# ZhendongWang6/Uformer

Hardware: AMD Instinct MI355X
Metric: restored images/sec (256x256, Uformer-B) (higher is better)
Workload: dtype bf16

## Files before the change

uformer_amd/csrc/uf_attnblk.hip:

```cpp
#include <stdlib.h>

#include <atomic>
#include <type_traits>

#include "uf_internal.h"

namespace uf {
namespace {

struct AttnBlkParams {
    float* x; int ld;
    float* xo; int ldo;
    const float* gamma; const float* beta; const float* modulator;
    const void* Wqkv; const float* bqkv;
    const float* rpb_tab;
    const void* Wp; const float* bp;
    const float* gamma2; const float* beta2;
    const void* W1; const float* b1;
    void* h1;
    const float* drop;
    void* s_xn; void* s_q; void* s_k; void* s_vt; void* s_o; void* s_z;
    int n_windows, H, W, shift;
    float qscale;
    float qscale_plain;
    unsigned long long* tbuf;
};

constexpr float LOG2E = 1.4426950408889634f;

#ifndef UF_P1_OFFSET
#define UF_P1_OFFSET 0
#endif
#ifndef UF_FC1_OFFSET
#define UF_FC1_OFFSET 0
#endif
#ifndef UF_STAGGER
#define UF_STAGGER 0
#endif
#ifndef UF_SETPRIO
#define UF_SETPRIO 0
#endif
#define UF_PRIO_UP() do { if (UF_SETPRIO) __builtin_amdgcn_s_setprio(1); } while (0)
#define UF_PRIO_DN() do { if (UF_SETPRIO) __builtin_amdgcn_s_setprio(0); } while (0)
#ifndef UF_ABL
#define UF_ABL 0
#endif
#ifndef UF_NT
#define UF_NT 0
#endif
#ifndef UF_LN_ROTATE
#define UF_LN_ROTATE 0
#endif
#ifndef UF_LN_WIDE
#define UF_LN_WIDE 1
#endif
#ifndef UF_QKV_RING
#define UF_QKV_RING 3
#endif
#ifndef UF_PROJ_RING
#define UF_PROJ_RING 3
#endif
#ifndef UF_FC1_RING
#define UF_FC1_RING 5
#endif
#ifndef UF_HOIST
#define UF_HOIST 7
#endif
template <int C> constexpr bool hoist_on() { return (C <= 128 && (UF_HOIST & 1)) || (C == 256 && (UF_HOIST & 2)) || (C == 512 && (UF_HOIST & 4)); }

#ifndef UF_ATTN_LR_DEFAULT
#define UF_ATTN_LR_DEFAULT 0
#endif
template <typename T> struct FragFromAcc {
    static __device__ __forceinline__ void make(Frag<T>& f, f32x4 a, f32x4 b) {
        f.v = u32x4{pack2<T>(a[0], a[1]), pack2<T>(a[2], a[3]), pack2<T>(b[0], b[1]), pack2<T>(b[2], b[3])};
    }
};
template <> struct FragFromAcc<float> {
    static __device__ __forceinline__ void make(Frag<float>& f, f32x4 a, f32x4 b) { f.lo = a; f.hi = b; }
};

template <typename T> __device__ __forceinline__ void wfrag_load(Frag<T>& f, const T* p) {
    if constexpr (UF_ABL == 6 && sizeof(T) == 2) { const unsigned v = 0x3c003c00u ^ (unsigned)(uintptr_t)p; f.v = u32x4{v, v, v, v}; }
    else load_frag(f, p);
}
template <typename T> __device__ __forceinline__ void afrag_load(Frag<T>& f, const T* p) {
    if constexpr (UF_ABL == 7 && sizeof(T) == 2) { const unsigned v = 0x3c003c00u ^ (unsigned)(uintptr_t)p; f.v = u32x4{v, v, v, v}; }
    else load_frag(f, p);
}

template <typename T> __device__ __forceinline__ void pin_frag(Frag<T>& f) {
    if constexpr (sizeof(T) == 2) asm volatile("" : "+v"(f.v));
}

template <int N> __device__ __forceinline__ float tree_sum(float* v) {
    static_assert((N & (N - 1)) == 0, "power of two");
#pragma unroll
    for (int w = 1; w < N; w *= 2)
#pragma unroll
        for (int i = 0; i < N; i += 2 * w) v[i] += v[i + w];
    return v[0];
}

template <typename T, int C, int WAVES, int UW = 4, bool ACT = true>
struct Fc1Walk {
    static_assert(UW == 4 || UW == 2, "units of 64 x 64 or 64 x 32");
    static constexpr int SZ = sizeof(T), KS = C / 32, RING = KS >= 8 ? UF_FC1_RING : (KS >= 4 ? 4 : 3), N4 = 4 * C, UNITS = N4 / (16 * UW);
    const T* wrow[UW];
    Frag<T> wf[RING][UW];
    const T* W1;
    int lane;
    __device__ __forceinline__ void wload(int ks, int slot) {
#pragma unroll
        for (int i = 0; i < UW; ++i) wfrag_load(wf[slot][i], wrow[i] + ks * 512);
    }
    __device__ __forceinline__ void unit_prefetch(int u) {
#pragma unroll
        for (int i = 0; i < UW; ++i) wrow[i] = W1 + ((size_t)(u * UW + i) * KS * 64 + lane) * 8;
#pragma unroll
        for (int s = 0; s < RING - 1; ++s)
            if (s < KS) wload(s, s);
    }
    __device__ __forceinline__ void first(const T* W1_, int wave, int lane_) {
        W1 = W1_; lane = lane_;
        if (wave < UNITS) unit_prefetch(wave);
    }
    __device__ __forceinline__ void run(const char* Xn, int SA, const float* b1, T* h1, const WinGeom& geo, int wave) {
    static_assert(SZ == 2, "direct-store epilogue packs pairs of a 2-byte type");
    const int fr = lane & 15, fg = lane >> 4;
    size_t rowoff[4];
#pragma unroll
    for (int j = 0; j < 4; ++j) rowoff[j] = (size_t)window_token(geo, j * 16 + fr) * N4;
    if (WAVES == 8 && UF_FC1_OFFSET > 0 && wave >= 4) __builtin_amdgcn_s_sleep(UF_FC1_OFFSET * (C / 256) > 127 ? 127 : UF_FC1_OFFSET * (C / 256));
#pragma unroll 1
    for (int u = wave; u < UNITS; u += WAVES) {
        const int nbase = u * 16 * UW;
        f32x4 acc[UW][4];
#pragma unroll
        for (int i = 0; i < UW; ++i)
#pragma unroll
            for (int j = 0; j < 4; ++j) acc[i][j] = f32x4{0.f, 0.f, 0.f, 0.f};
        const char* arow = Xn + fr * SA + fg * 8 * SZ;
        Frag<T> af[2][4];
        auto aload = [&](int ks, int slot) {
#pragma unroll
            for (int j = 0; j < 4; ++j) afrag_load(af[slot][j], reinterpret_cast<const T*>(arow + j * 16 * SA + ks * 32 * SZ));
        };
        aload(0, 0);
        f32x4 bv[UW];
#pragma unroll
        for (int i = 0; i < UW; ++i) bv[i] = *reinterpret_cast<const f32x4*>(b1 + nbase + i * 16 + fg * 4);
#pragma unroll
        for (int ks = 0; ks < KS; ++ks) {
            if (ks + RING - 1 < KS) wload(ks + RING - 1, (ks + RING - 1) % RING);
            if (ks + 1 < KS) aload(ks + 1, (ks + 1) & 1);
            __builtin_amdgcn_sched_barrier(0);
            UF_PRIO_UP();
#pragma unroll
            for (int i = 0; i < UW; ++i)
#pragma unroll
                for (int j = 0; j < 4; ++j) mma16(acc[i][j], wf[ks % RING][i], af[ks & 1][j]);
            UF_PRIO_DN();
            __builtin_amdgcn_sched_barrier(0);
        }
        if (u + WAVES < UNITS) unit_prefetch(u + WAVES);
        __builtin_amdgcn_sched_barrier(0);
#pragma unroll
        for (int j = 0; j < 4; ++j) {
#pragma unroll
            for (int ip = 0; ip < UW; ip += 2) {
                f32x4 va = acc[ip][j] + bv[ip], vb = acc[ip + 1][j] + bv[ip + 1];
                if (UF_ABL != 8 && ACT) { gelu4<T>(va); gelu4<T>(vb); }
                const unsigned a0 = pack2<T>(va[0], va[1]), a1 = pack2<T>(va[2], va[3]);
                const unsigned c0 = pack2<T>(vb[0], vb[1]), c1 = pack2<T>(vb[2], vb[3]);
                const u32x2_t s0 = __builtin_amdgcn_permlane16_swap(a0, c0, false, false);
                const u32x2_t s1 = __builtin_amdgcn_permlane16_swap(a1, c1, false, false);
                const int n = nbase + (ip + (fg & 1)) * 16 + (fg >> 1) * 8;
                if (UF_ABL == 4) asm volatile("" :: "v"(s0[0]), "v"(s1[0]), "v"(s0[1]), "v"(s1[1]), "v"(h1 + rowoff[j] + n));
                else if (UF_NT & 1) __builtin_nontemporal_store(u32x4{s0[0], s1[0], s0[1], s1[1]}, reinterpret_cast<u32x4*>(h1 + rowoff[j] + n));
                else *reinterpret_cast<u32x4*>(h1 + rowoff[j] + n) = u32x4{s0[0], s1[0], s0[1], s1[1]};
            }
        }
    }
    }
};

struct NoWalk {
    template <typename... A> __device__ __forceinline__ void first(A...) {}
    template <typename... A> __device__ __forceinline__ void run(A...) {}
};

template <typename T, int C, int NT, int LR = 0, int TR = 0>
__global__ __launch_bounds__(NT, LR == 3 ? 3 : (LR == 1 ? (C <= 32 ? 5 : (C == 64 ? 4 : 3)) : ((sizeof(T) == 2 && C <= 32) ? 4 : ((sizeof(T) == 2 && C == 64) ? 3 : 2)))) void attn_block_kernel(const AttnBlkParams p) {
    constexpr bool ST = LR == 3;
    constexpr int SZ = sizeof(T);
    constexpr int WAVES = NT / 64;
    constexpr int HEADS = C / 32;
    constexpr int SA = C * SZ + 16;
    constexpr int KS = C / 32;
    constexpr int QT = HEADS >= 4 ? 4 : HEADS;
    constexpr int UNITS = HEADS * (4 / QT);
    extern __shared__ __attribute__((aligned(16))) char smem[];
    char* Xn = smem;
    char* Os = ST ? smem : smem + 64 * SA;
    float* Tab = reinterpret_cast<float*>(smem + (ST ? 1 : 2) * 64 * SA);
    float* Red = Tab + HEADS * 225;
    float* Bq = Red + 2 * WAVES * 64;

    const int tid = threadIdx.x, lane = tid & 63;
    const int wave = __builtin_amdgcn_readfirstlane(tid >> 6);
    const int fr = lane & 15, fg = lane >> 4;
    const int bw = blockIdx.x;
    const WinGeom geo = window_geom(bw, p.H, p.W, p.shift);
    auto stamp = [&](int k) {
        if (p.tbuf && lane == 0 && (bw & 63) == 0) p.tbuf[((bw >> 6) * WAVES + wave) * 16 + k] = __builtin_readcyclecounter();
    };
    stamp(0);
    Census census; census.begin();
    if (UF_STAGGER > 0 && ((blockIdx.x >> 8) & 1)) {
#pragma unroll
        for (int k = 0; k < UF_STAGGER; ++k) __builtin_amdgcn_s_sleep(127);
    }

    constexpr int NTABV = HEADS * 225 + 4 * C, NTAB = (NTABV + NT - 1) / NT;
    float tabv[NTAB];
#pragma unroll
    for (int k = 0; k < NTAB; ++k) {
        int i = tid + k * NT;
        i = i < NTABV ? i : NTABV - 1;
        const float* src = i < HEADS * 225 ? p.rpb_tab + i : (i < HEADS * 225 + 3 * C ? p.bqkv + (i - HEADS * 225) : p.bp + (i - HEADS * 225 - 3 * C));
        tabv[k] = *src;
    }
    constexpr bool HOIST = hoist_on<C>() && SZ == 2;
    constexpr int WR = (SZ == 2 && C >= 256) ? UF_QKV_RING : ((SZ == 2 && C >= 128) ? 3 : 2);
    const T* Wqkv = reinterpret_cast<const T*>(p.Wqkv);
    const T* wrow[6];
    Frag<T> wf[WR][LR ? 2 : 6];
    auto wload = [&](int ks, int slot) {
#pragma unroll
        for (int i = 0; i < 6; ++i) wfrag_load(wf[slot][i], wrow[i] + ks * 512);
    };
    auto wload2 = [&](int g, int slot) {
        const int pj = g / KS, ks = g - pj * KS, base = pj == 0 ? 2 : (pj == 1 ? 4 : 0);
#pragma unroll
        for (int i = 0; i < 2; ++i) wfrag_load(wf[slot][i], wrow[base + i] + ks * 512);
    };
    auto unit_weights = [&](int u) {
        const int h = u / (4 / QT);
#pragma unroll
        for (int i = 0; i < 6; ++i) wrow[i] = Wqkv + ((size_t)((i >> 1) * (C / 16) + h * 2 + (i & 1)) * KS * 64 + lane) * 8;
#pragma unroll
        for (int pf = 0; pf < WR - 1; ++pf) {
            if constexpr (LR) { if (pf < 3 * KS) wload2(pf, pf); }
            else { if (pf < KS) wload(pf, pf); }
        }
    };
    if constexpr (HOIST) {
        if (wave < UNITS) unit_weights(wave);
    }
    {
        constexpr int LPR = UF_LN_WIDE ? ((C / 16) < 8 ? 8 : (C / 16)) : ((C / 4) < 64 ? (C / 4) : 64);
        constexpr int V4 = C / (4 * LPR);
        constexpr int RPP = NT / LPR;
        constexpr int NP = 64 / RPP;
        constexpr int U0 = (16 / V4) < NP ? (16 / V4) : NP;
        constexpr int U = (ST && U0 > 2) ? 2 : U0;
        static_assert(NP >= 1 && NP % U == 0, "pass batching");
        const int sub = tid % LPR;
        static_assert((U & (U - 1)) == 0, "U is a power of two");
        const int rot = UF_LN_ROTATE ? bw : 0;
#pragma unroll 1
        for (int r0 = 0; r0 < 64; r0 += RPP * U) {
            f32x4 v[U][V4], md[U][V4];
#pragma unroll
            for (int u = 0; u < U; ++u) {
                const int src = window_token(geo, r0 + ((u + rot) & (U - 1)) * RPP + tid / LPR);
#pragma unroll
                for (int i = 0; i < V4; ++i) {
                    if (UF_ABL == 1) v[u][i] = f32x4{(float)src, (float)i, (float)sub, 1.0f};
                    else if (UF_NT & 4) v[u][i] = __builtin_nontemporal_load(reinterpret_cast<const f32x4*>(p.x + (size_t)src * p.ld + (i * LPR + sub) * 4));
                    else v[u][i] = *reinterpret_cast<const f32x4*>(p.x + (size_t)src * p.ld + (i * LPR + sub) * 4);
                }
            }
            if (p.modulator && UF_ABL != 3) {
#pragma unroll
                for (int u = 0; u < U; ++u) {
                    const int row = r0 + ((u + rot) & (U - 1)) * RPP + tid / LPR;
#pragma unroll
                    for (int i = 0; i < V4; ++i) md[u][i] = *reinterpret_cast<const f32x4*>(p.modulator + (size_t)row * C + (i * LPR + sub) * 4);
                }
            } else {
#pragma unroll
                for (int u = 0; u < U; ++u)
#pragma unroll
                    for (int i = 0; i < V4; ++i) md[u][i] = f32x4{0.f, 0.f, 0.f, 0.f};
            }
            f32x4 gm[V4], bt[V4];
#pragma unroll
            for (int i = 0; i < V4; ++i) {
                gm[i] = *reinterpret_cast<const f32x4*>(p.gamma + (i * LPR + sub) * 4);
                bt[i] = *reinterpret_cast<const f32x4*>(p.beta + (i * LPR + sub) * 4);
            }
#pragma unroll
            for (int u = 0; u < U; ++u) {
                const int row = r0 + ((u + rot) & (U - 1)) * RPP + tid / LPR;
                float sum = 0.f;
#pragma unroll
                for (int i = 0; i < V4; ++i) sum += (v[u][i][0] + v[u][i][1]) + (v[u][i][2] + v[u][i][3]);
                sum = allreduce<RedSum, LPR>(sum);
                const float mean = sum * (1.0f / C);
                float sq = 0.f;
#pragma unroll
                for (int i = 0; i < V4; ++i) {
                    v[u][i] -= mean;
                    sq += (v[u][i][0] * v[u][i][0] + v[u][i][1] * v[u][i][1]) + (v[u][i][2] * v[u][i][2] + v[u][i][3] * v[u][i][3]);
                }
                sq = allreduce<RedSum, LPR>(sq);
                float rstd;
                if constexpr (SZ == 2) rstd = __builtin_amdgcn_rsqf(sq * (1.0f / C) + 1e-5f);
                else rstd = 1.0f / sqrtf(sq * (1.0f / C) + 1e-5f);
#pragma unroll
                for (int i = 0; i < V4; ++i) {
                    const int c = (i * LPR + sub) * 4;
                    f32x4 y = v[u][i] * rstd * gm[i] + bt[i] + md[u][i];
                    if (UF_ABL == 2) y = v[u][i];
                    store4(reinterpret_cast<T*>(Xn + row * SA) + c, y);
                }
            }
        }
    }
#pragma unroll
    for (int k = 0; k < NTAB; ++k) {
        const int i = tid + k * NT;
        if (i < HEADS * 225) Tab[i] = tabv[k] * LOG2E;
        else if (i < HEADS * 225 + 4 * C) Bq[i - HEADS * 225] = tabv[k];
    }
    stamp(1);
    lds_barrier();
    stamp(2);
    auto tile_out = [&](const char* tile, void* dst, bool token_order) {
        constexpr int PPR = C * SZ / 16;
#pragma unroll 4
        for (int i = tid; i < 64 * PPR; i += NT) {
            const int r = i / PPR, pc = i - r * PPR;
            const size_t row = token_order ? (size_t)window_token(geo, r) : (size_t)bw * 64 + r;
            *reinterpret_cast<u32x4*>(reinterpret_cast<char*>(dst) + (row * C * SZ + pc * 16)) = *reinterpret_cast<const u32x4*>(tile + r * SA + pc * 16);
        }
    };
    if constexpr (TR) tile_out(Xn, p.s_xn, false);

    const int nWc = p.W >> 3, nW = (p.H >> 3) * nWc;
    const int wi = bw % nW;
    const bool last_r = p.shift > 0 && (wi / nWc) == (p.H >> 3) - 1;
    const bool last_c = p.shift > 0 && (wi % nWc) == nWc - 1;

    if (WAVES == 8 && UF_P1_OFFSET > 0 && wave >= 4) __builtin_amdgcn_s_sleep(UF_P1_OFFSET * (C / 256) > 127 ? 127 : UF_P1_OFFSET * (C / 256));
    constexpr int UPW = (UNITS + WAVES - 1) / WAVES;
    static_assert(!ST || (SZ == 2 && UNITS % WAVES == 0), "single-tile form: 2-byte operands, every wave owns the same number of heads");
    unsigned opk[ST ? UPW : 1][QT][4];
    auto unit = [&](const int u, const int ui) __attribute__((always_inline)) {
        const int h = u / (4 / QT), q0 = (u % (4 / QT)) * QT;
        Frag<T> qf[QT], kf[4], vtf[2][2];
        if constexpr (LR) {
            if constexpr (!HOIST) unit_weights(u);
            Frag<T> af[2][4];
            auto aload2 = [&](int g, int slot) {
                const int pj = g / KS, ks = g - pj * KS;
                if (pj < 2 || QT == 4) {
#pragma unroll
                    for (int j = 0; j < 4; ++j) afrag_load(af[slot][j], reinterpret_cast<const T*>(Xn + (j * 16 + fr) * SA + (ks * 32 + fg * 8) * SZ));
                } else {
#pragma unroll
                    for (int j = 0; j < QT; ++j) afrag_load(af[slot][j], reinterpret_cast<const T*>(Xn + ((q0 + j) * 16 + fr) * SA + (ks * 32 + fg * 8) * SZ));
                }
            };
            aload2(0, 0);
            const f32x4 bk0 = *reinterpret_cast<const f32x4*>(Bq + C + h * 32 + fg * 4), bk1 = *reinterpret_cast<const f32x4*>(Bq + C + h * 32 + 16 + fg * 4);
            {
                f32x4 ak[2][4];
#pragma unroll
                for (int i = 0; i < 2; ++i)
#pragma unroll
                    for (int j = 0; j < 4; ++j) ak[i][j] = f32x4{0.f, 0.f, 0.f, 0.f};
#pragma unroll
                for (int ks = 0; ks < KS; ++ks) {
                    const int g = ks;
                    if (g + WR - 1 < 3 * KS) wload2(g + WR - 1, (g + WR - 1) % WR);
                    aload2(g + 1, (g + 1) & 1);
                    __builtin_amdgcn_sched_barrier(0);
#pragma unroll
                    for (int i = 0; i < 2; ++i)
#pragma unroll
                        for (int j = 0; j < 4; ++j) mma16(ak[i][j], wf[g % WR][i], af[g & 1][j]);
                    __builtin_amdgcn_sched_barrier(0);
                }
#pragma unroll
                for (int j = 0; j < 4; ++j) { FragFromAcc<T>::make(kf[j], ak[0][j] + bk0, ak[1][j] + bk1); if constexpr (ST) pin_frag(kf[j]); }
            }
            {
                f32x4 av[2][4];
#pragma unroll
                for (int i = 0; i < 2; ++i)
#pragma unroll
                    for (int j = 0; j < 4; ++j) av[i][j] = f32x4{0.f, 0.f, 0.f, 0.f};
#pragma unroll
                for (int ks = 0; ks < KS; ++ks) {
                    const int g = KS + ks;
                    if (g + WR - 1 < 3 * KS) wload2(g + WR - 1, (g + WR - 1) % WR);
                    aload2(g + 1, (g + 1) & 1);
                    __builtin_amdgcn_sched_barrier(0);
#pragma unroll
                    for (int i = 0; i < 2; ++i)
#pragma unroll
                        for (int j = 0; j < 4; ++j) mma16(av[i][j], af[g & 1][j], wf[g % WR][i]);
                    __builtin_amdgcn_sched_barrier(0);
                }
                const float bv0 = Bq[2 * C + h * 32 + fr], bv1 = Bq[2 * C + h * 32 + 16 + fr];
#pragma unroll
                for (int sk = 0; sk < 2; ++sk) {
                    FragFromAcc<T>::make(vtf[0][sk], av[0][2 * sk] + bv0, av[0][2 * sk + 1] + bv0);
                    FragFromAcc<T>::make(vtf[1][sk], av[1][2 * sk] + bv1, av[1][2 * sk + 1] + bv1);
                    if constexpr (ST) { pin_frag(vtf[0][sk]); pin_frag(vtf[1][sk]); }
                }
            }
            {
                f32x4 aq[2][QT];
#pragma unroll
                for (int i = 0; i < 2; ++i)
#pragma unroll
                    for (int j = 0; j < QT; ++j) aq[i][j] = f32x4{0.f, 0.f, 0.f, 0.f};
#pragma unroll
                for (int ks = 0; ks < KS; ++ks) {
                    const int g = 2 * KS + ks;
                    if (g + WR - 1 < 3 * KS) wload2(g + WR - 1, (g + WR - 1) % WR);
                    if (ks + 1 < KS) aload2(g + 1, (g + 1) & 1);
                    __builtin_amdgcn_sched_barrier(0);
#pragma unroll
                    for (int i = 0; i < 2; ++i)
#pragma unroll
                        for (int j = 0; j < QT; ++j) mma16(aq[i][j], wf[g % WR][i], af[g & 1][j]);
                    __builtin_amdgcn_sched_barrier(0);
                }
                if (u == wave) stamp(3);
                if constexpr (HOIST) {
                    if (u + WAVES < UNITS) unit_weights(u + WAVES);
                }
                const f32x4 bq0 = *reinterpret_cast<const f32x4*>(Bq + h * 32 + fg * 4), bq1 = *reinterpret_cast<const f32x4*>(Bq + h * 32 + 16 + fg * 4);
#pragma unroll
                for (int j = 0; j < QT; ++j) FragFromAcc<T>::make(qf[j], (aq[0][j] + bq0) * p.qscale, (aq[1][j] + bq1) * p.qscale);
            }
        } else {
        f32x4 aq[2][QT], ak[2][4], av[2][4];
#pragma unroll
        for (int i = 0; i < 2; ++i) {
#pragma unroll
            for (int j = 0; j < QT; ++j) aq[i][j] = f32x4{0.f, 0.f, 0.f, 0.f};
#pragma unroll
            for (int j = 0; j < 4; ++j) { ak[i][j] = f32x4{0.f, 0.f, 0.f, 0.f}; av[i][j] = f32x4{0.f, 0.f, 0.f, 0.f}; }
        }
        Frag<T> af[2][4];
        Frag<T> afq[2][QT < 4 ? QT : 1];
        if constexpr (!HOIST) unit_weights(u);
        auto aload = [&](int ks, int slot) {
#pragma unroll
            for (int j = 0; j < 4; ++j) afrag_load(af[slot][j], reinterpret_cast<const T*>(Xn + (j * 16 + fr) * SA + (ks * 32 + fg * 8) * SZ));
            if constexpr (QT < 4) {
#pragma unroll
                for (int j = 0; j < QT; ++j)
                    afrag_load(afq[slot][j], reinterpret_cast<const T*>(Xn + ((q0 + j) * 16 + fr) * SA + (ks * 32 + fg * 8) * SZ));
            }
        };
        aload(0, 0);
#pragma unroll
        for (int ks = 0; ks < KS; ++ks) {
            if (ks + WR - 1 < KS) wload(ks + WR - 1, (ks + WR - 1) % WR);
            if (ks + 1 < KS) aload(ks + 1, (ks + 1) & 1);
            __builtin_amdgcn_sched_barrier(0);
            const int s = ks & 1, sw = ks % WR;
            UF_PRIO_UP();
#pragma unroll
            for (int i = 0; i < 2; ++i) {
#pragma unroll
                for (int j = 0; j < QT; ++j) {
                    if constexpr (QT < 4) mma16(aq[i][j], wf[sw][i], afq[s][j]);
                    else mma16(aq[i][j], wf[sw][i], af[s][j]);
                }
#pragma unroll
                for (int j = 0; j < 4; ++j) mma16(ak[i][j], wf[sw][2 + i], af[s][j]);
#pragma unroll
                for (int j = 0; j < 4; ++j) mma16(av[i][j], af[s][j], wf[sw][4 + i]);
            }
            UF_PRIO_DN();
            __builtin_amdgcn_sched_barrier(0);
        }
        if (u == wave) stamp(3);
        if constexpr (HOIST) {
            if (u + WAVES < UNITS) unit_weights(u + WAVES);
        }
        {
            const f32x4 bq0 = *reinterpret_cast<const f32x4*>(Bq + h * 32 + fg * 4), bq1 = *reinterpret_cast<const f32x4*>(Bq + h * 32 + 16 + fg * 4);
            const f32x4 bk0 = *reinterpret_cast<const f32x4*>(Bq + C + h * 32 + fg * 4), bk1 = *reinterpret_cast<const f32x4*>(Bq + C + h * 32 + 16 + fg * 4);
            const float bv0 = Bq[2 * C + h * 32 + fr], bv1 = Bq[2 * C + h * 32 + 16 + fr];
#pragma unroll
            for (int j = 0; j < QT; ++j) FragFromAcc<T>::make(qf[j], (aq[0][j] + bq0) * p.qscale, (aq[1][j] + bq1) * p.qscale);
#pragma unroll
            for (int j = 0; j < 4; ++j) FragFromAcc<T>::make(kf[j], ak[0][j] + bk0, ak[1][j] + bk1);
#pragma unroll
            for (int sk = 0; sk < 2; ++sk) {
                FragFromAcc<T>::make(vtf[0][sk], av[0][2 * sk] + bv0, av[0][2 * sk + 1] + bv0);
                FragFromAcc<T>::make(vtf[1][sk], av[1][2 * sk] + bv1, av[1][2 * sk + 1] + bv1);
            }
            if constexpr (TR && SZ == 2) {
                const size_t wh = (size_t)bw * HEADS + h;
                T* qb = reinterpret_cast<T*>(p.s_q) + wh * 2048;
#pragma unroll
                for (int j = 0; j < QT; ++j) {
                    store4(qb + ((q0 + j) * 16 + fr) * 32 + fg * 4, (aq[0][j] + bq0) * p.qscale_plain);
                    store4(qb + ((q0 + j) * 16 + fr) * 32 + 16 + fg * 4, (aq[1][j] + bq1) * p.qscale_plain);
                }
                if (q0 == 0) {
                    T* kb = reinterpret_cast<T*>(p.s_k) + wh * 2048;
                    T* vb = reinterpret_cast<T*>(p.s_vt) + wh * 2048;
#pragma unroll
                    for (int j = 0; j < 4; ++j) {
                        *reinterpret_cast<u32x2*>(kb + (j * 16 + fr) * 32 + fg * 4) = u32x2{kf[j].v[0], kf[j].v[1]};
                        *reinterpret_cast<u32x2*>(kb + (j * 16 + fr) * 32 + 16 + fg * 4) = u32x2{kf[j].v[2], kf[j].v[3]};
                    }
#pragma unroll
                    for (int i = 0; i < 2; ++i)
#pragma unroll
                        for (int sk = 0; sk < 2; ++sk) {
                            *reinterpret_cast<u32x2*>(vb + (i * 16 + fr) * 64 + (2 * sk) * 16 + fg * 4) = u32x2{vtf[i][sk].v[0], vtf[i][sk].v[1]};
                            *reinterpret_cast<u32x2*>(vb + (i * 16 + fr) * 64 + (2 * sk + 1) * 16 + fg * 4) = u32x2{vtf[i][sk].v[2], vtf[i][sk].v[3]};
                        }
                }
            }
        }
        }
        f32x4 s[4][QT];
#pragma unroll
        for (int kt = 0; kt < 4; ++kt)
#pragma unroll
            for (int j = 0; j < QT; ++j) {
                s[kt][j] = f32x4{0.f, 0.f, 0.f, 0.f};
                mma16(s[kt][j], kf[kt], qf[j]);
            }
        if (u == wave) stamp(8);
        {
            const int dyc = (fr >> 3) - (fg >> 1);
            const int xb = 7 - (fr & 7) + 4 * (fg & 1);
            const float* th = Tab + h * 225 + xb;
            auto tb_row = [&](int d) {
                int row = 2 * (q0 + d - 3) + dyc + 7;
                row = row < 0 ? 0 : (row > 14 ? 14 : row);
                const float* tr = th + row * 15;
                return f32x4{tr[0], tr[1], tr[2], tr[3]};
            };
            if constexpr (ST) {
#pragma unroll
                for (int d = 0; d < 7; ++d) {
                    const f32x4 tbd = tb_row(d);
#pragma unroll
                    for (int j = 0; j < QT; ++j)
                        if (j + 3 - d >= 0 && j + 3 - d < 4) s[j + 3 - d][j] += tbd;
                    __builtin_amdgcn_sched_barrier(0);
                }
            } else {
                f32x4 tb[7];
#pragma unroll
                for (int d = 0; d < 7; ++d) tb[d] = tb_row(d);
#pragma unroll
                for (int j = 0; j < QT; ++j)
#pragma unroll
                    for (int kt = 0; kt < 4; ++kt) s[kt][j] += tb[j - kt + 3];
            }
        }
        if (last_r || last_c) {
#pragma unroll
            for (int j = 0; j < QT; ++j) {
                const int qi = (q0 + j) * 16 + fr;
                const bool q_lo_y = (qi >> 3) >= 4, q_lo_x = (qi & 7) >= 4;
#pragma unroll
                for (int kt = 0; kt < 4; ++kt) {
                    const int k0 = kt * 16 + fg * 4;
                    const bool dy = last_r && (((k0 >> 3) >= 4) != q_lo_y);
#pragma unroll
                    for (int r = 0; r < 4; ++r) {
                        const bool k_lo_x = ((k0 & 7) + r) >= 4;
                        if (dy || (last_c && (k_lo_x != q_lo_x))) s[kt][j][r] += -100.0f * LOG2E;
                    }
                }
            }
        }
        float inv[QT];
#pragma unroll
        for (int j = 0; j < QT; ++j) {
            float mx = -3.0e38f;
#pragma unroll
            for (int kt = 0; kt < 4; ++kt)
#pragma unroll
                for (int r = 0; r < 4; ++r) mx = fmaxf(mx, s[kt][j][r]);
            mx = red_xor32<RedMax>(red_xor16<RedMax>(mx));
            float sum = 0.f;
#pragma unroll
            for (int kt = 0; kt < 4; ++kt)
#pragma unroll
                for (int r = 0; r < 4; ++r) {
                    const float e = UF_ABL == 9 ? s[kt][j][r] - mx : __builtin_amdgcn_exp2f(s[kt][j][r] - mx);
                    s[kt][j][r] = e;
                    sum += e;
                }
            sum = red_xor32<RedSum>(red_xor16<RedSum>(sum));
            inv[j] = 1.0f / sum;
        }
        if (u == wave) stamp(9);
        f32x4 o[2][QT];
#pragma unroll
        for (int dt = 0; dt < 2; ++dt)
#pragma unroll
            for (int j = 0; j < QT; ++j) o[dt][j] = f32x4{0.f, 0.f, 0.f, 0.f};
#pragma unroll
        for (int sk = 0; sk < 2; ++sk)
#pragma unroll
            for (int j = 0; j < QT; ++j) {
                Frag<T> pf;
                FragFromAcc<T>::make(pf, s[2 * sk][j], s[2 * sk + 1][j]);
                mma16(o[0][j], vtf[0][sk], pf);
                mma16(o[1][j], vtf[1][sk], pf);
            }
        if (u == wave) stamp(10);
#pragma unroll
        for (int j = 0; j < QT; ++j) {
            if constexpr (ST) {
                const f32x4 oa = o[0][j] * inv[j], ob = o[1][j] * inv[j];
                opk[ui][j][0] = pack2<T>(oa[0], oa[1]); opk[ui][j][1] = pack2<T>(oa[2], oa[3]);
                opk[ui][j][2] = pack2<T>(ob[0], ob[1]); opk[ui][j][3] = pack2<T>(ob[2], ob[3]);
                asm volatile("" : "+v"(opk[ui][j][0]), "+v"(opk[ui][j][1]), "+v"(opk[ui][j][2]), "+v"(opk[ui][j][3]));
            } else {
                T* orow = reinterpret_cast<T*>(Os + ((q0 + j) * 16 + fr) * SA) + h * 32 + fg * 4;
                store4(orow, o[0][j] * inv[j]);
                store4(orow + 16, o[1][j] * inv[j]);
            }
        }
        if (u == wave) stamp(4);
    };
    if constexpr (ST) {
#pragma unroll
        for (int ui = 0; ui < UPW; ++ui) unit(wave + ui * WAVES, ui);
        lds_barrier();
#pragma unroll
        for (int ui = 0; ui < UPW; ++ui) {
            const int u = wave + ui * WAVES, h = u / (4 / QT), q0 = (u % (4 / QT)) * QT;
#pragma unroll
            for (int j = 0; j < QT; ++j) {
                char* orow = Os + ((q0 + j) * 16 + fr) * SA + (h * 32 + fg * 4) * SZ;
                *reinterpret_cast<u32x2*>(orow) = u32x2{opk[ui][j][0], opk[ui][j][1]};
                *reinterpret_cast<u32x2*>(orow + 16 * SZ) = u32x2{opk[ui][j][2], opk[ui][j][3]};
            }
        }
    } else {
#pragma unroll 1
        for (int u = wave; u < UNITS; u += WAVES) unit(u, 0);
    }
    stamp(5);
    std::conditional_t<SZ == 2, Fc1Walk<T, C, WAVES, LR ? 2 : 4, TR == 0>, NoWalk> fc1w;
    {
        constexpr int WN = (C / 16) < WAVES ? (C / 16) : WAVES, WM = WAVES / WN;
        constexpr int TNW = (C / 16) / WN, TMW = (4 / WM) > 0 ? (4 / WM) : 1;
        static_assert(WM <= 4, "more waves than 16-row tiles");
        const int wm = wave / WN, wn = wave % WN;
        const T* Wp = reinterpret_cast<const T*>(p.Wp);
        f32x4 acc[TNW][TMW];
#pragma unroll
        for (int i = 0; i < TNW; ++i)
#pragma unroll
            for (int j = 0; j < TMW; ++j) acc[i][j] = f32x4{0.f, 0.f, 0.f, 0.f};
        constexpr int PR = SZ == 2 ? (KS >= 8 ? UF_PROJ_RING : 3) : 2;
        Frag<T> wf[PR][TNW], af[2][TMW];
        auto wload = [&](int ks, int slot) {
#pragma unroll
            for (int i = 0; i < TNW; ++i) wfrag_load(wf[slot][i], Wp + (((size_t)(wn * TNW + i) * KS + ks) * 64 + lane) * 8);
        };
        auto aload = [&](int ks, int slot) {
#pragma unroll
            for (int j = 0; j < TMW; ++j) afrag_load(af[slot][j], reinterpret_cast<const T*>(Os + ((wm * TMW + j) * 16 + fr) * SA + (ks * 32 + fg * 8) * SZ));
        };
        float* xrow[TMW];
        float* xorow[TMW];
#pragma unroll
        for (int j = 0; j < TMW; ++j) {
            const size_t tok = (size_t)window_token(geo, (wm * TMW + j) * 16 + fr);
            xrow[j] = p.x + tok * p.ld;
            xorow[j] = p.xo + tok * p.ldo;
        }
        constexpr bool PRE = SZ == 2 && !ST;
        f32x4 res[PRE ? TNW : 1][PRE ? TMW : 1];
        auto proj_requests = [&]() {
#pragma unroll
            for (int pf = 0; pf < PR - 1; ++pf)
                if (pf < KS) wload(pf, pf);
            if constexpr (PRE) {
#pragma unroll
                for (int i = 0; i < TNW; ++i) {
                    const int n = (wn * TNW + i) * 16 + fg * 4;
#pragma unroll
                    for (int j = 0; j < TMW; ++j) res[i][j] = *reinterpret_cast<const f32x4*>(xrow[j] + n);
                }
            }
        };
        if constexpr (HOIST) proj_requests();
        lds_barrier();
        stamp(6);
        if constexpr (TR) tile_out(Os, p.s_o, false);
        if constexpr (!HOIST) proj_requests();
        aload(0, 0);
#pragma unroll
        for (int ks = 0; ks < KS; ++ks) {
            if (ks + PR - 1 < KS) wload(ks + PR - 1, (ks + PR - 1) % PR);
            if (ks + 1 < KS) aload(ks + 1, (ks + 1) & 1);
            __builtin_amdgcn_sched_barrier(0);
            UF_PRIO_UP();
#pragma unroll
            for (int i = 0; i < TNW; ++i)
#pragma unroll
                for (int j = 0; j < TMW; ++j) mma16(acc[i][j], wf[ks % PR][i], af[ks & 1][j]);
            UF_PRIO_DN();
            __builtin_amdgcn_sched_barrier(0);
        }
        stamp(7);
        if constexpr (SZ == 2 && HOIST) {
            if (p.h1) fc1w.first(reinterpret_cast<const T*>(p.W1), wave, lane);
        }
        const float dscale = p.drop ? p.drop[geo.img] : 1.0f;
#pragma unroll
        for (int j = 0; j < TMW; ++j) {
            float* xr = xrow[j];
            float* xw = xorow[j];
#pragma unroll
            for (int i = 0; i < TNW; ++i) {
                const int n = (wn * TNW + i) * 16 + fg * 4;
                const f32x4 b = *reinterpret_cast<const f32x4*>(Bq + 3 * C + n);
                if constexpr (PRE) acc[i][j] = res[i][j] + (acc[i][j] + b) * dscale;
                else acc[i][j] = *reinterpret_cast<const f32x4*>(xr + n) + (acc[i][j] + b) * dscale;
                if (UF_ABL == 5) asm volatile("" :: "v"(acc[i][j][0]), "v"(acc[i][j][1]), "v"(acc[i][j][2]), "v"(acc[i][j][3]), "v"(xw + n));
                else if (UF_NT & 2) __builtin_nontemporal_store(acc[i][j], reinterpret_cast<f32x4*>(xw + n));
                else *reinterpret_cast<f32x4*>(xw + n) = acc[i][j];
            }
        }
        if constexpr (SZ == 2) {
            if (p.h1) {
                float mean[TMW], rstd[TMW];
#pragma unroll
                for (int pass = 0; pass < 2; ++pass) {
#pragma unroll
                    for (int j = 0; j < TMW; ++j) {
                        float part[TNW];
#pragma unroll
                        for (int i = 0; i < TNW; ++i) {
                            if (pass == 0) part[i] = (acc[i][j][0] + acc[i][j][1]) + (acc[i][j][2] + acc[i][j][3]);
                            else {
                                const f32x4 d = acc[i][j] - mean[j];
                                part[i] = (d[0] * d[0] + d[1] * d[1]) + (d[2] * d[2] + d[3] * d[3]);
                            }
                            part[i] = red_xor32<RedSum>(red_xor16<RedSum>(part[i]));
                        }
                        const float sacc = tree_sum<TNW>(part);
                        if (fg == 0) Red[(pass * WAVES + wave) * 64 + (wm * TMW + j) * 16 + fr] = sacc;
                    }
                    lds_barrier();
#pragma unroll
                    for (int j = 0; j < TMW; ++j) {
                        float wsum[WN];
#pragma unroll
                        for (int w2 = 0; w2 < WN; ++w2) wsum[w2] = Red[(pass * WAVES + wm * WN + w2) * 64 + (wm * TMW + j) * 16 + fr];
                        const float tot = tree_sum<WN>(wsum);
                        if (pass == 0) mean[j] = tot * (1.0f / C);
                        else rstd[j] = 1.0f / sqrtf(tot * (1.0f / C) + 1e-5f);
                    }
                }
#pragma unroll
                for (int i = 0; i < TNW; ++i) {
                    const int n = (wn * TNW + i) * 16 + fg * 4;
                    const f32x4 g2 = *reinterpret_cast<const f32x4*>(p.gamma2 + n), b2 = *reinterpret_cast<const f32x4*>(p.beta2 + n);
#pragma unroll
                    for (int j = 0; j < TMW; ++j)
                        store4(reinterpret_cast<T*>(Xn + ((wm * TMW + j) * 16 + fr) * SA) + n, (acc[i][j] - mean[j]) * rstd[j] * g2 + b2);
                }
            }
        }
    }
    if constexpr (SZ == 2) {
        if (p.h1) {
            lds_barrier();
            stamp(11);
            if constexpr (TR) tile_out(Xn, p.s_z, true);
            if constexpr (!HOIST) fc1w.first(reinterpret_cast<const T*>(p.W1), wave, lane);
            fc1w.run(Xn, SA, p.b1, reinterpret_cast<T*>(p.h1), geo, wave);
            stamp(12);
        }
    }
    census.end(p.tbuf, bw);
}

template <typename T, int C, int NT, int LR = 0, int TR = 0>
int launch_one(const AttnBlkParams& p, hipStream_t st) {
    constexpr int smem = (LR == 3 ? 1 : 2) * 64 * (C * (int)sizeof(T) + 16) + (C / 32) * 225 * 4 + 2 * (NT / 64) * 64 * 4 + 4 * C * 4;
    static_assert(smem <= 160 * 1024, "LDS budget");
    auto kern = attn_block_kernel<T, C, NT, LR, TR>;
    static bool lds_done[64] = {};
    if (int rc = ensure_dynamic_lds(reinterpret_cast<const void*>(kern), smem, lds_done, "attn_block")) return rc;
    char name[96] = "";
    if (timing_enabled())
        snprintf(name, sizeof(name), "attn_block%s_%s_c%d_nt%d %dx%d", TR ? "_train" : (p.h1 ? "_fc1" : ""), TypeName<T>::s, C, NT, p.n_windows * 64, C);
    const double M = (double)p.n_windows * 64;
    const double fc1_flops = p.h1 ? 2.0 * M * C * 4.0 * C : 0.0, fc1_bytes = p.h1 ? M * 4.0 * C * sizeof(T) + 4.0 * C * C * sizeof(T) : 0.0;
    {
        const double side_bytes = TR ? 6.0 * M * C * sizeof(T) : 0.0;
        ScopedTimer tm(name, 2.0 * M * C * (4.0 * C + 128.0) + fc1_flops, M * C * 8.0 + 4.0 * C * C * sizeof(T) + fc1_bytes + side_bytes, st);
        hipLaunchKernelGGL(kern, dim3(p.n_windows), dim3(NT), smem, st, p);
    }
    return check_launch("attn_block");
}

}

static std::atomic<unsigned long long*> g_tbuf{nullptr};
void debug_set_tbuf(void* p) { g_tbuf.store((unsigned long long*)p, std::memory_order_release); }
unsigned long long* debug_get_tbuf() { return g_tbuf.load(std::memory_order_acquire); }

bool attn_block_supported(const uf_block_params* bp, const float* user_mask, uf_dtype dtype, int C, int heads) {
    if (!bp->rpb_tab || user_mask) return false;
    if (heads <= 0 || C != heads * 32) return false;
    if (dtype_half(dtype)) return C == 32 || C == 64 || C == 128 || C == 256 || C == 512;
    return C == 32 || C == 64 || C == 128 || C == 256;
}

int launch_attn_block(const uf_block_params* bp, float* x, int ld, int B, int H, int W, int C, uf_dtype dtype, void* h1_out, hipStream_t st, const float* drop,
                      float* xo, int ldo) {
    AttnBlkParams p{};
    p.drop = drop;
    p.x = x; p.ld = ld;
    p.xo = xo ? xo : x; p.ldo = xo ? ldo : ld; p.gamma = bp->norm1_w; p.beta = bp->norm1_b; p.modulator = bp->modulator;
    p.Wqkv = bp->wqkv_fm; p.bqkv = bp->bqkv; p.rpb_tab = bp->rpb_tab;
    p.Wp = bp->wproj_fm; p.bp = bp->bproj;
    p.gamma2 = bp->norm2_w; p.beta2 = bp->norm2_b; p.W1 = bp->w1_fm; p.b1 = bp->b1;
    p.h1 = dtype_half(dtype) ? h1_out : nullptr;
    p.n_windows = B * (H / 8) * (W / 8); p.H = H; p.W = W; p.shift = bp->shift;
    p.qscale = (float)(1.0 / sqrt(32.0)) * LOG2E;
    p.tbuf = debug_get_tbuf();

    const int forced = variant("attn", -1);
    const int lr = (forced >= 0 && forced <= 2) ? forced : (forced == 3 ? 0 : (C == 32 ? 2 : ((C == 128 && p.n_windows >= 4096) ? 1 : 0)));
    const bool st256 = forced == 3;
#define UF_AB(TT, CV, NTV) return launch_one<TT, CV, NTV>(p, st)
#define UF_AB_HALF(TT)                                                                                                              \
        switch (C) {                                                                                                                    \
            case 32: if (lr == 1) return launch_one<TT, 32, 256, 1>(p, st); if (lr == 2) return launch_one<TT, 32, 256, 2>(p, st); UF_AB(TT, 32, 256);      \
            case 64: if (lr == 1) return launch_one<TT, 64, 256, 1>(p, st); if (lr == 2) return launch_one<TT, 64, 256, 2>(p, st); UF_AB(TT, 64, 256);      \
            case 128: if (lr == 1) return launch_one<TT, 128, 256, 1>(p, st); if (lr == 2) return launch_one<TT, 128, 256, 2>(p, st); UF_AB(TT, 128, 256);                                                                                              \
            case 256:                                                                                                                   \
                if (p.n_windows <= 256) UF_AB(TT, 256, 512);    \
                if (st256) return launch_one<TT, 256, 256, 3>(p, st);          \
                UF_AB(TT, 256, 256);                                                                                                    \
            case 512: UF_AB(TT, 512, 512);                                                                                              \
        }
    if (dtype == UF_BF16) {
        UF_AB_HALF(bf16)
    } else if (dtype == UF_F16) {
        UF_AB_HALF(f16)
    } else {
        switch (C) {
            case 32: UF_AB(float, 32, 256);
            case 64: UF_AB(float, 64, 256);
            case 128: UF_AB(float, 128, 256);
            case 256: UF_AB(float, 256, 256);
        }
    }
#undef UF_AB_HALF
#undef UF_AB
    set_error("attn_block: unsupported C=%d for dtype %d", C, (int)dtype);
    return UF_ERR_UNSUPPORTED;
}


int launch_attn_block_train(const uf_block_params* bp, const float* x, int ld, float* x1, int ld1, int B, int H, int W, int C, uf_dtype dtype, const float* drop,
                            void* xn, void* q, void* k, void* vt, void* o, void* z, void* a1, hipStream_t st) {
    AttnBlkParams p{};
    p.drop = drop;
    p.x = const_cast<float*>(x); p.ld = ld;
    p.xo = x1; p.ldo = ld1; p.gamma = bp->norm1_w; p.beta = bp->norm1_b; p.modulator = bp->modulator;
    p.Wqkv = bp->wqkv_fm; p.bqkv = bp->bqkv; p.rpb_tab = bp->rpb_tab;
    p.Wp = bp->wproj_fm; p.bp = bp->bproj;
    p.gamma2 = bp->norm2_w; p.beta2 = bp->norm2_b; p.W1 = bp->w1_fm; p.b1 = bp->b1;
    p.h1 = a1;
    p.s_xn = xn; p.s_q = q; p.s_k = k; p.s_vt = vt; p.s_o = o; p.s_z = z;
    p.n_windows = B * (H / 8) * (W / 8); p.H = H; p.W = W; p.shift = bp->shift;
    p.qscale_plain = (float)(1.0 / sqrt(32.0));
    p.qscale = p.qscale_plain * LOG2E;
    p.tbuf = debug_get_tbuf();
#define UF_ABT(TT)                                                                                          \
        switch (C) {                                                                                        \
            case 32: return launch_one<TT, 32, 256, 0, 1>(p, st);                                           \
            case 64: return launch_one<TT, 64, 256, 0, 1>(p, st);                                           \
            case 128: return launch_one<TT, 128, 256, 0, 1>(p, st);                                         \
            case 256:                                                                                       \
                if (p.n_windows <= 256) return launch_one<TT, 256, 512, 0, 1>(p, st);                       \
                return launch_one<TT, 256, 256, 0, 1>(p, st);                                               \
            case 512: return launch_one<TT, 512, 512, 0, 1>(p, st);                                         \
        }
    if (dtype == UF_BF16) {
        UF_ABT(bf16)
    } else if (dtype == UF_F16) {
        UF_ABT(f16)
    }
#undef UF_ABT
    set_error("attn_block (training form): unsupported C=%d for dtype %d (bf16 / f16 operands, C = 32 ... 512)", C, (int)dtype);
    return UF_ERR_UNSUPPORTED;
}

}
```

Baseline: 2492.

## Add single-wave attention block variant for C=32 with barrier elision

Adds a 64-thread (one wave) and 128-thread variant of the fused window attention block, with a configurable query-tiles-per-unit parameter. It selects the single-wave path by default when C is 32 and there are at least 8192 windows. With one wave, workgroup barriers become an LDS waitcnt and the cross-wave LayerNorm reduction is done in registers. The aim is to cut synchronization cost and raise the number of resident workgroups for the shallow encoder and decoder stages. The trade-off is that each wave does all heads' work serially, so per-block latency goes up.

```diff
diff --git a/uformer_amd/csrc/uf_attnblk.hip b/uformer_amd/csrc/uf_attnblk.hip
--- a/uformer_amd/csrc/uf_attnblk.hip
+++ b/uformer_amd/csrc/uf_attnblk.hip
@@ -190,15 +190,24 @@
     template <typename... A> __device__ __forceinline__ void run(A...) {}
 };
 
-template <typename T, int C, int NT, int LR = 0, int TR = 0>
-__global__ __launch_bounds__(NT, LR == 3 ? 3 : (LR == 1 ? (C <= 32 ? 5 : (C == 64 ? 4 : 3)) : ((sizeof(T) == 2 && C <= 32) ? 4 : ((sizeof(T) == 2 && C == 64) ? 3 : 2)))) void attn_block_kernel(const AttnBlkParams p) {
+template <typename T, int C, int NT, int LR> constexpr int attn_waves_per_simd() {
+    if (NT <= 128) return C <= 32 ? 3 : 2;
+    return LR == 3 ? 3 : (LR == 1 ? (C <= 32 ? 5 : (C == 64 ? 4 : 3)) : ((sizeof(T) == 2 && C <= 32) ? 4 : ((sizeof(T) == 2 && C == 64) ? 3 : 2)));
+}
+template <int WAVES> __device__ __forceinline__ void phase_barrier() {
+    if constexpr (WAVES == 1) asm volatile("s_waitcnt lgkmcnt(0)" ::: "memory");
+    else lds_barrier();
+}
+template <typename T, int C, int NT, int LR = 0, int TR = 0, int QTP = 0>
+__global__ __launch_bounds__(NT, (attn_waves_per_simd<T, C, NT, LR>())) void attn_block_kernel(const AttnBlkParams p) {
     constexpr bool ST = LR == 3;
     constexpr int SZ = sizeof(T);
     constexpr int WAVES = NT / 64;
     constexpr int HEADS = C / 32;
     constexpr int SA = C * SZ + 16;
     constexpr int KS = C / 32;
-    constexpr int QT = HEADS >= 4 ? 4 : HEADS;
+    constexpr int QT = QTP ? QTP : (HEADS >= 4 ? 4 : HEADS);
+    static_assert(QT == 1 || QT == 2 || QT == 4, "query tiles per unit");
     constexpr int UNITS = HEADS * (4 / QT);
     extern __shared__ __attribute__((aligned(16))) char smem[];
     char* Xn = smem;
@@ -336,7 +345,7 @@
         else if (i < HEADS * 225 + 4 * C) Bq[i - HEADS * 225] = tabv[k];
     }
     stamp(1);
-    lds_barrier();
+    phase_barrier<WAVES>();
     stamp(2);
     auto tile_out = [&](const char* tile, void* dst, bool token_order) {
         constexpr int PPR = C * SZ / 16;
@@ -647,7 +656,7 @@
     if constexpr (ST) {
 #pragma unroll
         for (int ui = 0; ui < UPW; ++ui) unit(wave + ui * WAVES, ui);
-        lds_barrier();
+        phase_barrier<WAVES>();
 #pragma unroll
         for (int ui = 0; ui < UPW; ++ui) {
             const int u = wave + ui * WAVES, h = u / (4 / QT), q0 = (u % (4 / QT)) * QT;
@@ -709,7 +718,7 @@
             }
         };
         if constexpr (HOIST) proj_requests();
-        lds_barrier();
+        phase_barrier<WAVES>();
         stamp(6);
         if constexpr (TR) tile_out(Os, p.s_o, false);
         if constexpr (!HOIST) proj_requests();
@@ -765,9 +774,13 @@
                             part[i] = red_xor32<RedSum>(red_xor16<RedSum>(part[i]));
                         }
                         const float sacc = tree_sum<TNW>(part);
-                        if (fg == 0) Red[(pass * WAVES + wave) * 64 + (wm * TMW + j) * 16 + fr] = sacc;
+                        if constexpr (WN == 1) {
+                            if (pass == 0) mean[j] = sacc * (1.0f / C);
+                            else rstd[j] = 1.0f / sqrtf(sacc * (1.0f / C) + 1e-5f);
+                        } else if (fg == 0) Red[(pass * WAVES + wave) * 64 + (wm * TMW + j) * 16 + fr] = sacc;
                     }
-                    lds_barrier();
+                    if constexpr (WN > 1) {
+                    phase_barrier<WAVES>();
 #pragma unroll
                     for (int j = 0; j < TMW; ++j) {
                         float wsum[WN];
@@ -777,6 +790,7 @@
                         if (pass == 0) mean[j] = tot * (1.0f / C);
                         else rstd[j] = 1.0f / sqrtf(tot * (1.0f / C) + 1e-5f);
                     }
+                    }
                 }
 #pragma unroll
                 for (int i = 0; i < TNW; ++i) {
@@ -791,7 +805,7 @@
     }
     if constexpr (SZ == 2) {
         if (p.h1) {
-            lds_barrier();
+            phase_barrier<WAVES>();
             stamp(11);
             if constexpr (TR) tile_out(Xn, p.s_z, true);
             if constexpr (!HOIST) fc1w.first(reinterpret_cast<const T*>(p.W1), wave, lane);
@@ -802,11 +816,11 @@
     census.end(p.tbuf, bw);
 }
 
-template <typename T, int C, int NT, int LR = 0, int TR = 0>
+template <typename T, int C, int NT, int LR = 0, int TR = 0, int QTP = 0>
 int launch_one(const AttnBlkParams& p, hipStream_t st) {
     constexpr int smem = (LR == 3 ? 1 : 2) * 64 * (C * (int)sizeof(T) + 16) + (C / 32) * 225 * 4 + 2 * (NT / 64) * 64 * 4 + 4 * C * 4;
     static_assert(smem <= 160 * 1024, "LDS budget");
-    auto kern = attn_block_kernel<T, C, NT, LR, TR>;
+    auto kern = attn_block_kernel<T, C, NT, LR, TR, QTP>;
     static bool lds_done[64] = {};
     if (int rc = ensure_dynamic_lds(reinterpret_cast<const void*>(kern), smem, lds_done, "attn_block")) return rc;
     char name[96] = "";
@@ -852,11 +866,18 @@
     const int forced = variant("attn", -1);
     const int lr = (forced >= 0 && forced <= 2) ? forced : (forced == 3 ? 0 : (C == 32 ? 2 : ((C == 128 && p.n_windows >= 4096) ? 1 : 0)));
     const bool st256 = forced == 3;
+    const int nt_small = forced == 4 ? 64 : (forced == 5 ? 128 : ((forced < 0 && C == 32 && p.n_windows >= 8192) ? 64 : 0));
 #define UF_AB(TT, CV, NTV) return launch_one<TT, CV, NTV>(p, st)
 #define UF_AB_HALF(TT)                                                                                                              \
         switch (C) {                                                                                                                    \
-            case 32: if (lr == 1) return launch_one<TT, 32, 256, 1>(p, st); if (lr == 2) return launch_one<TT, 32, 256, 2>(p, st); UF_AB(TT, 32, 256);      \
-            case 64: if (lr == 1) return launch_one<TT, 64, 256, 1>(p, st); if (lr == 2) return launch_one<TT, 64, 256, 2>(p, st); UF_AB(TT, 64, 256);      \
+            case 32:                                                                                                                    \
+                if (nt_small == 64) return launch_one<TT, 32, 64, 0, 0, 4>(p, st);          \
+                if (nt_small == 128) return launch_one<TT, 32, 128, 0, 0, 2>(p, st);                     \
+                if (lr == 1) return launch_one<TT, 32, 256, 1>(p, st); if (lr == 2) return launch_one<TT, 32, 256, 2>(p, st); UF_AB(TT, 32, 256);      \
+            case 64:                                                                                                                    \
+                if (nt_small == 64) return launch_one<TT, 64, 64, 0, 0, 4>(p, st);             \
+                if (nt_small == 128) return launch_one<TT, 64, 128, 0, 0, 4>(p, st);                            \
+                if (lr == 1) return launch_one<TT, 64, 256, 1>(p, st); if (lr == 2) return launch_one<TT, 64, 256, 2>(p, st); UF_AB(TT, 64, 256);      \
             case 128: if (lr == 1) return launch_one<TT, 128, 256, 1>(p, st); if (lr == 2) return launch_one<TT, 128, 256, 2>(p, st); UF_AB(TT, 128, 256);                                                                                              \
             case 256:                                                                                                                   \
                 if (p.n_windows <= 256) UF_AB(TT, 256, 512);    \
```

Measured after the change: 2525, median of 6. 1.01x the previous value.
